# moabarar/nemar

Measured on AMD Instinct MI355X. Metric: train images/sec (256x256 A/B pairs), higher is better.
Workload: dtype f32

## Files before the change

nemar_amd/csrc/conv.hip:

```cpp
#define NEMAR_CONV_HIP
#include "common.h"
#include "conv_exact.h"
#include "conv_call.h"
#include "conv_route.h"
#include "pack_plan.h"

#ifdef NEMAR_AB
extern int g_split16_ring3;
extern int g_split16_ksplit_cap;
extern int g_narrow_fwd4;
extern int g_wg_xreg;
extern int g_register_vec4;
extern int g_overlap_per_lane;
extern int g_histogram_per_lane;
void nemar_norm_planes_debug(int bits);
#endif

int nemar_narrow_fwd(const float* x, const float* w, const float* bias, float* y, int N, int C, int H, int W, int K, int R,
                     int pad, int border, int act, float slope, float* part, size_t part_floats, hipStream_t st);
int nemar_narrow_wgrad(const float* x, const float* gy, float* gw, int N, int C, int H, int W, int K, int R, int pad,
                       int border, float* part, hipStream_t st);
void nemar_wgrad2_launch(const float* x0, int C0, const float* x1, int C1, const float* gy, float* gw, float* gb, int N,
                         int H, int W, int K, int OH, int OW, int R, int S, int stride, int pad, int pad_mode,
                         int target_blocks, bool vec_ok, int dbg, float* part, hipStream_t st);
// ... 792 lines not shown
                                       (const float*)ring_buf, gx0 ? gx0 : gx1, H, W, pad, ring_len, band, planes);
            }
        }
    if (fold && !folded) {
        const float* const add = (gx0 && !gx1) ? call.addend : nullptr;
        fold_padded(padded, gx0 ? gx0 : gx1, H, W, pad, total, add, st);
        if (add) call.addend_done = true;
    }
    }
    }
    NEMAR_CHECK_LAUNCH(what);
    return NEMAR_OK;
}

NEMAR_API size_t nemar_conv2d_bwd_weight_workspace(int N, int C, int H, int W, int K, int OH, int OW, int R, int S, int stride, int pad) {
    if (N <= 0 || C <= 0 || K <= 0 || OH <= 0 || OW <= 0 || R <= 0 || S <= 0) return 0;
    return sizeof(float) * plan_wgrad({N, C, 0, H, W, K, R, S, stride, pad, BORDER_ZERO, OH, OW}, ConvFacts::canonical()).total;
}

static int conv2d_bwd_weight(ConvCall& call, const float* x0, int C0, const float* x1, int C1, const float* gy, float* gw,
                             float* gb, int N, int H, int W, int K, int OH, int OW, int R, int S, int stride,
                             int pad, int pad_mode, void* workspace, size_t ws_bytes, void* stream) {
    NEMAR_CLEAR_HIP_ERROR();
    NEMAR_REQUIRE(x0 && gy && gw, "conv2d_bwd_weight: null pointer");
    NEMAR_REQUIRE(C0 > 0 && C1 >= 0 && (C1 == 0 || x1), "conv2d_bwd_weight: bad channel split");
    NEMAR_REQUIRE(N > 0 && H > 0 && W > 0 && K > 0 && OH > 0 && OW > 0 && R > 0 && S > 0, "conv2d_bwd_weight: bad shape");
    NEMAR_REQUIRE(pad_mode == BORDER_ZERO || (pad < H && pad < W), "conv2d_bwd_weight: reflect pad too large");
    NEMAR_REQUIRE((long long)N * OH * OW < (1ll << 31) && (long long)(C0 + C1) * H * W < (1ll << 31),
                  "conv2d_bwd_weight: problem too large for 32-bit tile indexing");
    ConvFacts f = facts_of(call, nullptr, ACT_NONE, 0.f);
    f.part = g_deterministic != 0;
    f.gy_aligned = (reinterpret_cast<uintptr_t>(gy) & 15) == 0;
    f.part_aligned = (reinterpret_cast<uintptr_t>(workspace) & 15) == 0;
    const WgradPlan P = plan_wgrad({N, C0, C1, H, W, K, R, S, stride, pad, pad_mode, OH, OW}, f);
    float* part = nullptr;
    if (g_deterministic) {
        const size_t need = sizeof(float) * P.total;
        if (!workspace || ws_bytes < need) {
            nemar_set_error("conv2d_bwd_weight: workspace %zu < %zu", workspace ? ws_bytes : (size_t)0, need);
            return NEMAR_EWORKSPACE;
        }
        part = (float*)workspace;
    }
    hipStream_t st = (hipStream_t)stream;
    const int J = (C0 + C1) * R * S;
    const char* what = "conv2d_bwd_weight";
    g_last_route = P.route;
    switch (P.sub) {
    case WgradPlan::K7:
        if (!nemar_k7_wgrad(x0, gy, gw, gb, N, C0, H, W, K, pad_mode, part, st))
            bias_grad_slabs(gy, gb, part + P.bias_off, N, K, OH * OW, st);
        what = "conv2d_bwd_weight (7x7, 16-bit pipe)";
        break;
    case WgradPlan::NARROW:
        nemar_narrow_wgrad(x0, gy, gw, N, C0, H, W, K, R, pad, pad_mode, part, st);
        if (gb) bias_grad_slabs(gy, gb, part ? part + P.bias_off : nullptr, N, K, OH * OW, st);
        what = "conv2d_bwd_weight (narrow)";
        break;
    case WgradPlan::S16G:
        nemar_s16g_wgrad(x0, C0, x1, C1, gy, gw, gb, N, H, W, K, OH, OW, R, stride, pad_mode, part, g_dbg, st);
        what = "conv2d_bwd_weight (16-bit pipe, in-kernel split)";
        break;
    case WgradPlan::SPLIT16:
        call.bias_rode = gb && call.bias_partials;
        nemar_split16_wgrad(x0, gy, gw, N, C0, H, W, K, R, pad_mode == BORDER_REFLECT ? 1 : 0, call.scratch, part, g_xcd_map,
                            R == 3 ? call.src2_planes : nullptr, (R == 3 && pad_mode == BORDER_REFLECT) ? call.x_planes : nullptr,
                            call.src_max, call.src2_max, call.bias_rode ? call.bias_partials : nullptr, gb, st);
        if (gb && !call.bias_rode) bias_grad_slabs(gy, gb, part + P.bias_off, N, K, OH * OW, st);
        what = "conv2d_bwd_weight (split-16)";
        break;
    case WgradPlan::WGRAD2:
        nemar_wgrad2_launch(x0, C0, x1, C1, gy, gw, gb, N, H, W, K, OH, OW, R, S, stride, pad, pad_mode, g_wgrad_blocks,
                            g_wgrad != 2, g_dbg, part, st);
        what = "conv2d_bwd_weight (wide)";
        break;
    case WgradPlan::WGRAD2_PADDED_GY: {
        float* gyp = part + P.gyp_off;
        const long long total = (long long)N * K * P.ohv * OW;
        hipLaunchKernelGGL(pad_planes_kernel, dim3(nemar_stream_grid(total, 256)), dim3(256), 0, st, gy, gyp, OH * OW, P.ohv * OW, total);
        nemar_wgrad2_launch(x0, C0, x1, C1, gyp, gw, gb, N, H, W, K, P.ohv, OW, R, S, stride, pad, pad_mode, g_wgrad_blocks,
                            g_wgrad != 2, g_dbg, part, st);
        what = "conv2d_bwd_weight (wide, padded gy)";
        break;
    }
    case WgradPlan::LEGACY: {
        WgradParams p;
        p.src0 = x0; p.src1 = x1; p.C0 = C0; p.C1 = C1; p.Hs = H; p.Ws = W;
        p.gy = gy; p.K = K; p.OH = OH; p.OW = OW;
        p.gw = gw; p.gb = gb; p.J = J;
        p.N = N; p.P = N * OH * OW; p.sy = stride; p.sx = stride; p.R = R; p.S = S; p.pad = pad; p.border = pad_mode;
        p.fd_ohw = make_fastdiv(OH * OW); p.fd_ow = make_fastdiv(OW);
        p.dbg = g_dbg;
        p.pix_per_split = P.pix_per_split;
        p.part = part;
        p.partb = part ? part + P.bias_off : nullptr;
        const bool wide = K > 32;
        dim3 grid(nemar_cdiv(K, wide ? 128 : 32), nemar_cdiv(J, wide ? 128 : 256), P.splits), block(256);
        if (wide) hipLaunchKernelGGL((wgrad_kernel<2, 2, 2, 2>), grid, block, 0, st, p);
        else hipLaunchKernelGGL((wgrad_kernel<1, 4, 1, 2>), grid, block, 0, st, p);
        if (part) nemar_sum_partials_pair(part, (long long)K * J, P.splits, gw, (long long)K * J, gb ? p.partb : nullptr, K, P.splits, gb, K, true, st);
    }
    }
// ... 24 lines not shown
    if (key == 26) { g_s16g_wgrad_first = value != 0; return NEMAR_OK; }
    if (key == 27) { nemar_s16g_tune(0, value); return NEMAR_OK; }
    if (key == 29) { g_s16g_wgrad = value != 0; return NEMAR_OK; }
    if (key == 31) { nemar_norm_planes_debug(value); return NEMAR_OK; }
    if (key == 32) { g_split16_ring3 = value != 0; return NEMAR_OK; }
    if (key == 33) { g_k7 = value != 0; return NEMAR_OK; }
    if (key == 36) { g_split_act = value != 0; return NEMAR_OK; }
    if (key == 43) { g_fold_small = value != 0; return NEMAR_OK; }
    if (key == 37) { g_lds_claim = value; return NEMAR_OK; }
    if (key == 38) { g_wg_xreg = value != 0; return NEMAR_OK; }
    if (key == 39) { g_split16_ksplit_cap = value < 1 ? 1 : (value > 8 ? 8 : value); return NEMAR_OK; }
    if (key == 45) { g_overlap_per_lane = value != 0; return NEMAR_OK; }
    if (key == 46) { g_histogram_per_lane = value != 0; return NEMAR_OK; }
    if (key == 44) { g_register_vec4 = value != 0; return NEMAR_OK; }
    if (key == 47) { g_pointwise_rows = value != 0; return NEMAR_OK; }
    if (key == 35) { g_dual_gy = value != 0; return NEMAR_OK; }
    if (key == 34) { nemar_split16_wgrad_tune(value); return NEMAR_OK; }
    if (key == 30) { g_s16g_fold = value != 0; return NEMAR_OK; }
    if (key == 28) { nemar_s16g_tune(1, value); return NEMAR_OK; }
    if (key == 40) { nemar_s16g_tune(2, value); return NEMAR_OK; }
    if (key == 42) { nemar_s16g_tune(4, value); return NEMAR_OK; }
    if (key == 41) { nemar_s16g_tune(3, value); return NEMAR_OK; }
    if (key == 23) { g_split16_min_mmac = value < 0 ? 0 : value; return NEMAR_OK; }
    if (key == 21) { g_split16_variant = value == 3 ? 3 : 4; return NEMAR_OK; }
    if (key == 16) { g_adir = value != 0; return NEMAR_OK; }
    if (key == 17) { g_mt8 = value; return NEMAR_OK; }
    if (key == 19) { g_narrow_fwd4 = value != 0; return NEMAR_OK; }
    if (key == 18) { g_ring = (value == 4 || value == 5) ? value : 3; return NEMAR_OK; }
    if (key == 12) { g_ksplit = value != 0; return NEMAR_OK; }
    if (key == 11) { g_nl4_scalar = value != 0; return NEMAR_OK; }
    if (key == 10) { g_deep64 = value != 0; return NEMAR_OK; }
    if (key == 7) { g_ws2_mt = (value == 1 || value == 2 || value == 4) ? value : 0; return NEMAR_OK; }
    if (key == 5) { g_wgrad_blocks = value > 0 ? value : 512; return NEMAR_OK; }
    nemar_set_error("nemar_tune: unknown key %d", key);
    return NEMAR_EINVAL;
}
#endif

static DgradPlan usual_dgrad(int N, int C, int H, int W, int K, int R, int S, int stride, int pad, int pad_mode) {
    DgradPlan P{};
    if (N <= 0 || C <= 0 || H <= 0 || W <= 0 || K <= 0 || R <= 0 || S <= 0 || stride < 1) return P;
    return plan_dgrad({N, C, 0, H, W, K, R, S, stride, pad, pad_mode}, ConvFacts::canonical());
}
static bool fusable(const DgradPlan& P) { return P.gy_planes_need != 0 && P.split16_ksplit == 1; }

NEMAR_API size_t nemar_conv2d_scratch(int N, int H, int W, int K, int C, int R, int S, int stride, int pad) {
    if (N <= 0 || H <= 0 || W <= 0 || K <= 0 || C <= 0) return 0;
    return plan_arena_bytes({N, C, 0, H, W, K, R, S, stride, pad, BORDER_ZERO});
}

NEMAR_API size_t nemar_conv2d_gy_planes_bytes(int N, int C, int H, int W, int K, int R, int S, int stride, int pad, int pad_mode) {
    return usual_dgrad(N, C, H, W, K, R, S, stride, pad, pad_mode).gy_planes_need;
}

NEMAR_API int nemar_conv2d_bwd_data_fusable(int N, int C, int H, int W, int K, int R, int S, int stride, int pad, int pad_mode) {
    return fusable(usual_dgrad(N, C, H, W, K, R, S, stride, pad, pad_mode)) ? 1 : 0;
}

NEMAR_API int nemar_conv2d_bwd_data_addend_ok(int N, int C, int H, int W, int K, int R, int S, int stride, int pad, int pad_mode) {
    const DgradPlan P = usual_dgrad(N, C, H, W, K, R, S, stride, pad, pad_mode);
    if (fusable(P)) return 1;
    if (pad_mode != BORDER_REFLECT || pad <= 0 || stride != 1 || pad >= H || pad >= W || R != S || R == 7) return 0;
    return (P.fold16 || P.fold) && plan_arena_bytes({N, C, 0, H, W, K, R, S, stride, pad, BORDER_ZERO}) == 0 ? 1 : 0;
}

NEMAR_API int nemar_last_gy_planes(void) { return g_last_gy_planes; }
// ... 127 lines not shown
```

nemar_amd/csrc/conv_route.h:

```cpp
#pragma once
#ifndef NEMAR_CONV_HIP
#error "conv_route.h holds conv.hip's own switches: include it from conv.hip only"
#endif
#include "common.h"
#include "conv_exact.h"
#include "conv_split16.h"
#include "conv_s16g.h"
#include "conv_k7.h"

bool nemar_narrow_eligible(int K, int C1, int R, int S, int stride, int N, int OH, int OW);
int nemar_narrow_wgrad_splits(int N, int C, int OH, int OW);
bool nemar_wgrad2_eligible(int K, int OH, int OW, bool gy_aligned16);
void nemar_wgrad2_plan(int K, int J, int P, int target_blocks, int* splits_out, int* pix_per_split_out);

using namespace nemar_exact;

namespace {

static NEMAR_SWITCH(int, g_split16, 1);
static NEMAR_SWITCH(long long, g_split16_min_mmac, 2000);
static NEMAR_SWITCH(int, g_split16_variant, 4);
static NEMAR_SWITCH(int, g_k7, 1);
static NEMAR_SWITCH(int, g_s16g, 1);
static NEMAR_SWITCH(long long, g_s16g_min_mmac, 30);
static NEMAR_SWITCH(int, g_s16g_wgrad, 1);
static NEMAR_SWITCH(int, g_s16g_wgrad_first, 0);
static NEMAR_SWITCH(int, g_s16g_fold, 1);
static NEMAR_SWITCH(int, g_split_act, 1);
static NEMAR_SWITCH(int, g_fold_small, 1);
static NEMAR_SWITCH(int, g_dual_gy, 1);
static NEMAR_SWITCH(int, g_reflect_aux, 1);
static NEMAR_SWITCH(int, g_deterministic, 1);
static NEMAR_SWITCH(int, g_ksplit, 1);
static NEMAR_SWITCH(int, g_narrow, 1);
static NEMAR_SWITCH(int, g_wgrad, 0);
static NEMAR_SWITCH(int, g_wgrad_blocks, 512);

enum { ROUTE_EXACT = 0, ROUTE_NARROW = 1, ROUTE_SPLIT16 = 2, ROUTE_S16G = 3, ROUTE_K7 = 4 };

struct ConvShape {
    int N, C0, C1, H, W, K, R, S, stride, pad, pad_mode;
    int oh = 0, ow = 0;
    int C() const { return C0 + C1; }
    int OH() const { return oh ? oh : (H + 2 * pad - R) / stride + 1; }
    int OW() const { return ow ? ow : (W + 2 * pad - S) / stride + 1; }
    bool refl() const { return pad_mode == BORDER_REFLECT && pad > 0; }
    long long macs() const { return (long long)N * OH() * OW() * K * C() * R * S; }
};
struct ConvFacts {
    bool bias = false;
    int act = ACT_NONE;
    float slope = 0.f;
    bool gx0 = true, gx1 = false;
    bool part = true;
    size_t scratch_bytes = 0;
    size_t gy_planes_bytes = 0;
    bool gy_aligned = true, part_aligned = true;
    static ConvFacts canonical() { ConvFacts f; f.scratch_bytes = f.gy_planes_bytes = ~(size_t)0; return f; }
};

inline void grow(size_t& a, size_t b) { if (b > a) a = b; }
constexpr int WBK = 32;
constexpr int BIAS_CHUNK = 4096;

int small_problem_split(int M, int P, int Kred) {
    const TileChoice t = igemm_tile(M, P, nemar_cdiv(Kred, BK));
    if (t.bm == 128) return 1;
    const long long tiles = (long long)nemar_cdiv(M, t.bm) * nemar_cdiv(P, t.bn);
    const int stages = nemar_cdiv(Kred, BK);
    if (tiles >= 128 || stages < 16) return 1;
    int ks = nemar_cdiv(256, (int)tiles);
    if (ks > stages / 4) ks = stages / 4;
    return ks < 1 ? 1 : ks;
}

void fwd_taps(TapTable& t, int R, int S, int pad) {
    t.n = R * S;
    for (int r = 0; r < R; ++r)
        for (int s = 0; s < S; ++s) {
            t.dy[r * S + s] = (short)(r - pad);
            t.dx[r * S + s] = (short)(s - pad);
            t.dyx[r * S + s] = ((r - pad) << 16) | ((s - pad) & 0xffff);
            t.wofs[r * S + s] = r * S + s;
        }
}

void dgrad_taps(TapTable& t, int R, int S, int pad, int stride, int ph, int pw) {
    t.n = 0;
    for (int r = 0; r < R; ++r) {
        if ((ph + pad - r) % stride != 0) continue;
// ... 260 lines not shown
        L.route = ROUTE_EXACT; L.sub = DgradPlan::EXACT;
        L.narrow = g_narrow && stride == 1 && !L.fold && !f.bias && f.act == ACT_NONE && L.mskip == 0 && !f.gx1 && R - 1 - pad >= 0 &&
                   nemar_narrow_eligible(C, 0, R, S, 1, N, H, W);
        L.split = !L.narrow && L.ksplit > 1 && !f.bias && f.act == ACT_NONE && L.mskip == 0 &&
                  (L.fold ? (f.gx0 && !f.gx1) : (!f.gx1 || (f.gx0 && !L.ring)));
        L.aux_rows = !L.narrow && L.ring && g_reflect_aux && pad == 1 && R == 3 && S == 3 && H >= 4 && W >= 8;
    }
    return L;
}

void legacy_wgrad_plan(int K, int J, int P, int* splits_out, int* pix_per_split_out) {
    const bool wide = K > 32;
    const int BM = wide ? 128 : 32, BN = wide ? 128 : 256;
    const int mt = nemar_cdiv(K, BM), jt = nemar_cdiv(J, BN);
    int splits = nemar_cdiv(1024, mt * jt);
    const int max_splits = nemar_cdiv(P, WBK * 8);
    if (splits > max_splits) splits = max_splits;
    if (splits < 1) splits = 1;
    if (splits > 65535) splits = 65535;
    *pix_per_split_out = nemar_cdiv(nemar_cdiv(P, splits), WBK) * WBK;
    *splits_out = nemar_cdiv(P, *pix_per_split_out);
}
int padded_rows(int OH, int OW) {
    int ohv = OH;
    while ((ohv * OW) % 4) ++ohv;
    return ohv;
}
bool wgrad_pad_route(int K, int OH, int OW, int pad_mode) {
    return K > 4 && (OH * OW) % 4 != 0 && pad_mode == BORDER_ZERO && g_wgrad != 1;
}

struct WgradPlan {
    int route;
    enum Sub { K7, NARROW, S16G, SPLIT16, WGRAD2, WGRAD2_PADDED_GY, LEGACY } sub;
    size_t total, bias_off, gyp_off;
    int splits, pix_per_split, ohv;
};
WgradPlan plan_wgrad(const ConvShape& s, const ConvFacts& f) {
    WgradPlan P;
    const int N = s.N, C = s.C(), H = s.H, W = s.W, K = s.K, R = s.R, S = s.S, stride = s.stride, pad = s.pad, OH = s.OH(), OW = s.OW();
    const int J = C * R * S, Pix = N * OH * OW, ohv = padded_rows(OH, OW);
    const size_t slab = (size_t)K * J, bias_parts = (size_t)N * nemar_cdiv(OH * OW, BIAS_CHUNK) * K;
    int w2_splits, legacy_splits, pad_splits = 0, pps;
    nemar_wgrad2_plan(K, J, Pix, g_wgrad_blocks, &w2_splits, &pps);
    legacy_wgrad_plan(K, J, Pix, &legacy_splits, &P.pix_per_split);
    P.total = (size_t)(w2_splits > legacy_splits ? w2_splits : legacy_splits) * (slab + K);
    if ((OH * OW) % 4 != 0 && K > 4) {
        nemar_wgrad2_plan(K, J, N * ohv * OW, g_wgrad_blocks, &pad_splits, &pps);
        grow(P.total, (size_t)pad_splits * (slab + K) + 4 + (size_t)N * K * ohv * OW);
    }
    if (K <= 4) grow(P.total, (size_t)nemar_narrow_wgrad_splits(N, C, OH, OW) * slab + bias_parts);
    if (nemar_s16g_wgrad_eligible(N, C, 0, H, W, K, OH, OW, R, S, stride, pad, BORDER_ZERO))
        grow(P.total, (size_t)nemar_s16g_wgrad_slabs_max(N, C, K, OH, W, stride) * (slab + K));
    const bool k7 = nemar_k7_wgrad_eligible(N, C, H, W, K, R, S, stride, pad);
    if (k7) grow(P.total, nemar_k7_wgrad_floats(N, C, H, W, K) + bias_parts);
    const bool wide = wide_candidates(s).wgrad;
    if (wide) grow(P.total, (size_t)nemar_split16_wgrad_splits(N, C, H, W, K, R) * slab + bias_parts);
    const bool s16g_wg = g_s16g_wgrad && f.part && s16g_worth_it(s.macs()) &&
                         nemar_s16g_wgrad_eligible(N, s.C0, s.C1, H, W, K, OH, OW, R, S, stride, pad, s.pad_mode);
    const bool split16_wg = g_split16 && g_split16_variant == 4 && f.part && s.C1 == 0 && split16_worth_it(N, OH, OW, K, C, R, S) && wide &&
                            (R == 3 || s.pad_mode == BORDER_ZERO) && f.scratch_bytes &&
                            f.scratch_bytes >= nemar_split16_wgrad_scratch_bytes(N, C, H, W, K, R);
    P.bias_off = P.gyp_off = 0; P.splits = 0; P.ohv = ohv;
    if (g_k7 && f.part && s.C1 == 0 && k7) {
        P.route = ROUTE_K7; P.sub = WgradPlan::K7; P.bias_off = nemar_k7_wgrad_floats(N, C, H, W, K);
    } else if (nemar_narrow_eligible(K, s.C1, R, S, stride, N, OH, OW) && g_narrow) {
        P.route = ROUTE_NARROW; P.sub = WgradPlan::NARROW; P.bias_off = (size_t)nemar_narrow_wgrad_splits(N, s.C0, OH, OW) * slab;
    } else if (s16g_wg && (g_s16g_wgrad_first || !split16_wg)) {
        P.route = ROUTE_S16G; P.sub = WgradPlan::S16G;
    } else if (split16_wg) {
        P.route = ROUTE_SPLIT16; P.sub = WgradPlan::SPLIT16; P.bias_off = (size_t)nemar_split16_wgrad_splits(N, C, H, W, K, R) * slab;
    } else {
        P.route = ROUTE_EXACT;
        P.gyp_off = ((size_t)pad_splits * (slab + K) + 3) & ~(size_t)3;
        const bool padded_gy = f.part && wgrad_pad_route(K, OH, OW, s.pad_mode) && nemar_wgrad2_eligible(K, ohv, OW, f.part_aligned);
        if (g_wgrad != 1 && nemar_wgrad2_eligible(K, OH, OW, f.gy_aligned)) P.sub = WgradPlan::WGRAD2;
        else if (padded_gy) P.sub = WgradPlan::WGRAD2_PADDED_GY;
        else { P.sub = WgradPlan::LEGACY; P.splits = legacy_splits; P.bias_off = (size_t)legacy_splits * slab; }
    }
    return P;
}

size_t plan_arena_bytes(const ConvShape& s) {
    const int N = s.N, C = s.C(), H = s.H, W = s.W, K = s.K, R = s.R;
    if (!g_split16 || !split16_worth_it(N, H + 2 * s.pad - R + 1, W + 2 * s.pad - s.S + 1, K, C, R, s.S)) return 0;
    const WideCandidates c = wide_candidates(s);
    size_t b = c.fwd ? nemar_split16_scratch_total(N, H, W, K, C, H, W) : 0;
    if (c.dgrad) grow(b, nemar_split16_scratch_total(N, H, W, C, K, H, W));
    if (c.wgrad) grow(b, nemar_split16_wgrad_scratch_bytes(N, C, H, W, K, R));
    return b;
}

}
```

nemar_amd/csrc/conv_split16.h:

```cpp
#pragma once
#include <hip/hip_runtime.h>
#include <stddef.h>
#include "conv_call.h"

enum { SPLIT16_ZERO = 0, SPLIT16_REFLECT = 1, SPLIT16_DGRAD_REFLECT = 2 };

bool nemar_split16_eligible(int N, int H, int W, int M, int Cred, int R, int S, int stride, int pad, int mode, int variant);
size_t nemar_split16_scratch_bytes(int N, int Cred, int H, int W);
int nemar_split16_ksplit(int N, int H, int W, int M, int Cred);
size_t nemar_split16_scratch_total(int N, int H, int W, int M, int Cred, int OH, int OW);
size_t nemar_split16_pack_bytes(int M, int Cred, int KS);
void nemar_split16_pack(const float* w, void* packed, int K, int C, int KS, int dgrad, int variant, hipStream_t st);
struct Split16Done {
    bool dual_written;
    bool epilogue_fused;
};
Split16Done nemar_split16_conv(const float* src, const void* packed, const float* bias, float* dst, int N, int H, int W, int M, int Cred,
                               int KS, int src_pad, int Hs, int Ws_src, int OH, int OW, int mode, void* scratch, int xcd_map, int variant,
                               long long* tl, void* dual_g_out, MaxWords src_max, const void* ready_planes, int ready_kind,
                               const float* addend, void* out_max, hipStream_t st);

bool nemar_split16_wgrad_eligible(int N, int C, int H, int W, int K, int R, int S, int stride, int pad);
size_t nemar_split16_wgrad_scratch_bytes(int N, int C, int H, int W, int K, int KS);
int nemar_split16_wgrad_splits(int N, int C, int H, int W, int K, int KS);
#ifdef NEMAR_AB
void nemar_split16_wgrad_tune(int one_copy);
#endif
void nemar_sum_partials_pair(const float* part_a, long long stride_a, int splits_a, float* dst_a, long long n_a,
                             const float* part_b, long long stride_b, int splits_b, float* dst_b, long long n_b, bool accumulate, hipStream_t st);
void nemar_split16_wgrad(const float* x, const float* gy, float* gw, int N, int C, int H, int W, int K, int KS, int reflect,
                         void* scratch, float* part, int xcd_map, const void* g_planes, const void* x_planes, MaxWords x_max,
                         MaxWords gy_max, const float* bias_partials, float* gb, hipStream_t st);
size_t nemar_split16_wgrad_g_bytes(int N, int H, int W, int K, int KS);
void nemar_split16_dual_split(const float* gy, void* dplanes, void* gplanes, int N, int K, int H, int W, int mode, const unsigned* maxbits,
                              int mstride, hipStream_t st);
void nemar_sum_partials(const float* part, long long stride, int splits, float* dst, long long n, bool accumulate, hipStream_t st);
void nemar_sum_partials_two(const float* part, long long stride, int splits, float* d0, float* d1, int N, int C0, int C1, int HW, hipStream_t st);
void nemar_sum_partials_act(const float* part, long long stride, int splits, float* dst, long long n, int act, float slope, hipStream_t st);

void nemar_split16_absmax(const float* x, int samples, long long per, void* out, hipStream_t st);
const unsigned* nemar_split16_source_max(const float* src, int N, long long per, MaxWords hint, unsigned* own, int* stride, hipStream_t st);

void nemar_split16_timer(int on);
int nemar_split16_timer_read(double* total_ms, double* total_flop);
```

nemar_amd/csrc/conv_split16_wgrad.hip:

```cpp
#include "common.h"
#include "conv_split16.h"

namespace {

typedef float f32x16 __attribute__((ext_vector_type(16)));
typedef _Float16 f16x8 __attribute__((ext_vector_type(8)));
typedef unsigned u32x4 __attribute__((ext_vector_type(4)));

__device__ __forceinline__ float pow2_scale(unsigned maxbits) {
    const int e = (int)((maxbits >> 23) & 255u);
    if (e == 0 || e == 255) return 1.f;
    const int se = 127 + 11 - (e - 127);
    if (se < 1 || se > 254) return 1.f;
    return __builtin_bit_cast(float, (unsigned)se << 23);
}
__device__ __forceinline__ unsigned short f16_rn(float v) {
    const _Float16 h = (_Float16)v;
    return __builtin_bit_cast(unsigned short, h);
}
__device__ __forceinline__ void split2_f16(float v, unsigned short& h, unsigned short& l) {
    h = f16_rn(v);
    const float r = v - (float)__builtin_bit_cast(_Float16, h);
    l = f16_rn(r);
}
__device__ __forceinline__ u32x4 pack8(const unsigned short* b) {
    u32x4 o;
    o[0] = (unsigned)b[0] | ((unsigned)b[1] << 16);
    o[1] = (unsigned)b[2] | ((unsigned)b[3] << 16);
    o[2] = (unsigned)b[4] | ((unsigned)b[5] << 16);
    o[3] = (unsigned)b[6] | ((unsigned)b[7] << 16);
    return o;
}
__device__ __forceinline__ int mirror(int i, int n) { return i < 0 ? -i : (i >= n ? 2 * n - 2 - i : i); }

__device__ __forceinline__ void glds16(const u32x4* g, u32x4* lds) {
    __builtin_amdgcn_global_load_lds((const __attribute__((address_space(1))) void*)g,
                                     (__attribute__((address_space(3))) void*)lds, 16, 0, 0);
}
// ... 38 lines not shown
__global__ __launch_bounds__(256) void split_wgrad_x_kernel(const float* __restrict__ x, u32x4* __restrict__ out, int N, int C, int H,
                                                            int W, int Hp, int CPR, int reflect, long long total,
                                                            const unsigned* maxbits, int mstride) {
    __shared__ float tile[64][TW + 1];
    const int CBLK = C >> 6, FX = Hp * CPR;
    const int yp = blockIdx.x % Hp, cblk = (blockIdx.x / Hp) % CBLK, n = blockIdx.x / (Hp * CBLK);
    const float scale = pow2_scale(maxbits[n * mstride]);
    int y = yp - 1;
    bool rowok = yp < H + 2;
    if (reflect) y = mirror(min(y, H), H);
    else rowok = rowok && (unsigned)y < (unsigned)H;
    const float* src = x + (((size_t)n * C + cblk * 64) * H + (rowok ? y : 0)) * W;
    for (int i = threadIdx.x; i < 64 * W; i += 256) {
        const int cc = i / W, xs = i - cc * W;
        tile[cc][xs] = rowok ? src[(size_t)cc * H * W + xs] * scale : 0.f;
    }
    __syncthreads();
    const int cc = threadIdx.x & 63;
    for (int q = threadIdx.x >> 6; q < CPR; q += 4) {
        unsigned short h[8], l[8];
        float v[8];
#pragma unroll
        for (int e = 0; e < 8; ++e) {
            const int xs = q * 8 + e - 1;
            v[e] = tile[cc][min(max(reflect ? mirror(xs, W) : xs, 0), W - 1)];
        }
#pragma unroll
        for (int e = 0; e < 8; ++e) {
            const int xp = q * 8 + e;
            const bool ok = xp < W + 2 && (reflect || (unsigned)(xp - 1) < (unsigned)W);
            split2_f16(ok ? v[e] : 0.f, h[e], l[e]);
        }
        const size_t t = (((size_t)n * CBLK + cblk) * FX + (size_t)yp * CPR + q) * 64 + cc;
        out[t] = pack8(h);
        out[total + t] = pack8(l);
    }
}

template <int TW>
__global__ __launch_bounds__(256) void split_dual_kernel(const float* __restrict__ gy, u32x4* __restrict__ dpl, u32x4* __restrict__ gpl,
                                                         int N, int K, int H, int W, int Hg, int CPR, int reflect, long long dtotal,
                                                         long long gtotal, const unsigned* maxbits, int mstride) {
    __shared__ float tile[64][TW + 1];
    const int Hp = H + 4, Ws = W + 4, KBLK = K >> 6, CG = K >> 3, F = Hg * CPR;
    const int prow = blockIdx.x % Hp, kblk = (blockIdx.x / Hp) % KBLK, n = blockIdx.x / (Hp * KBLK);
    const float scale = pow2_scale(maxbits[n * mstride]);
    const bool img = prow >= 1 && prow <= H;
    int ya = 0, yb = -1;
    bool any = img;
    if (img) ya = prow - 1;
    else if (reflect && prow == H + 2) { ya = 0; yb = 2; any = true; }
    else if (reflect && prow == H + 3) { ya = H - 3; yb = H - 1; any = true; }
    const float* src = gy + ((size_t)n * K + kblk * 64) * H * W;
    for (int i = threadIdx.x; i < 64 * W; i += 256) {
        const int kk = i / W, x = i - kk * W;
        const float a = src[((size_t)kk * H + ya) * W + x];
        const float b = src[((size_t)kk * H + max(yb, 0)) * W + x];
        tile[kk][x] = any ? (yb >= 0 ? a + b : a) * scale : 0.f;
    }
    __syncthreads();
    for (int i = threadIdx.x; i < 8 * Ws; i += 256) {
        const int cgl = i / Ws, slot = i - cgl * Ws;
        int xa = -1, xb = -1;
        if (slot >= 1 && slot <= W) xa = slot - 1;
        else if (reflect && slot == W + 2) { xa = 0; xb = 2; }
        else if (reflect && slot == W + 3) { xa = W - 3; xb = W - 1; }
// ... 13 lines not shown
    const int grow = img ? prow - 1 : (prow == 0 ? H : prow);
    if (grow < Hg && (img || prow <= H + 2)) {
        const int kk = threadIdx.x & 63;
        for (int q = threadIdx.x >> 6; q < CPR; q += 4) {
            unsigned short h[8], l[8];
            float v[8];
#pragma unroll
            for (int e = 0; e < 8; ++e) v[e] = tile[kk][min(q * 8 + e, W - 1)];
#pragma unroll
            for (int e = 0; e < 8; ++e) split2_f16((img && q * 8 + e < W) ? v[e] : 0.f, h[e], l[e]);
            const size_t t = (((size_t)n * KBLK + kblk) * F + (size_t)grow * CPR + q) * 64 + kk;
            gpl[t] = pack8(h);
            gpl[gtotal + t] = pack8(l);
        }
    }
}

struct WgParams {
    const u32x4* G;
    const u32x4* X;
    float* part;
    int N, H, W, C, K;
    int CPR, F, FX, RB, spi;
    int KBLK, CBLK;
    long long gplane16, xplane16;
    const unsigned* gmax;
    const unsigned* xmax;
    int gstride, xstride;
    int xcd;
};

template <int KS, bool ONEG, bool XREG = false>
__global__ __launch_bounds__(256) void wgrad_split16_kernel(WgParams p) {
    static_assert(!XREG || (KS == 3 && ONEG), "XREG: instantiated and measured for the 3x3 one-copy form only");

    constexpr int GC = ONEG ? 1 : KS;
    constexpr int RING = 4, NCOL = 4 * GC + 4 * KS, NCP = NCOL / 4;
    constexpr int STAGE16 = NCOL * 64;
    constexpr int NMF = 3 * KS * KS, NSL = 2 * GC + 2 * KS + NCP;
    constexpr int NPV = KS / 2;
#ifdef NEMAR_HOST_EMULATION
    __shared__ __attribute__((aligned(16))) u32x4 smem[RING * STAGE16];
#else
    extern __shared__ __attribute__((aligned(16))) u32x4 smem[];
#endif
    const int tid = threadIdx.x, wid = __builtin_amdgcn_readfirstlane(tid >> 6), lane = tid & 63;
    const int tiles = p.KBLK * p.CBLK;
    int t = blockIdx.x;
    if (p.xcd) t = (t & 7) * ((int)gridDim.x >> 3) + (t >> 3);
    const int split = t / tiles, tile = t - split * tiles;
    const int kblk = tile / p.CBLK, cblk = tile - kblk * p.CBLK;
    const int n = split / p.spi, y0 = (split - n * p.spi) * p.RB;
    const int nsteps = p.RB * p.CPR / 2, f0 = y0 * p.CPR;

    const u32x4* csrc[NCP];
#pragma unroll
    for (int q = 0; q < NCP; ++q) {
        const int i = NCP * wid + q;
        if (i < 4 * GC) {
            const int s = i >> 2, pl = (i >> 1) & 1, ch = i & 1;
            csrc[q] = p.G + (size_t)(s * 2 + pl) * p.gplane16 + (((size_t)n * p.KBLK + kblk) * p.F + f0 + ch) * 64 + lane;
        } else {
            const int j = i - 4 * GC, r = j >> 2, pl = (j >> 1) & 1, ch = j & 1;
            csrc[q] = p.X + (size_t)pl * p.xplane16 + (((size_t)n * p.CBLK + cblk) * p.FX + f0 + r * p.CPR + ch) * 64 + lane;
        }
    }
#define WG_COPIES(stage_)                                                                                               \
// ... 244 lines not shown
    NEMAR_AB_ONLY(                                                                                                                 \
    else if (KS == 3)                                                                                                              \
        hipLaunchKernelGGL((split_wgrad_g_kernel<TW_, 3>), dim3(N * KBLK * Hg), dim3(256), 0, st, gy, (u32x4*)scratch, N, K, OHg, OWg, Hg, CPR, gtotal, \
                           gmax, gstride);                                                                                         \
    else                                                                                                                           \
        hipLaunchKernelGGL((split_wgrad_g_kernel<TW_, 4>), dim3(N * KBLK * Hg), dim3(256), 0, st, gy, (u32x4*)scratch, N, K, OHg, OWg, Hg, CPR, gtotal, \
                           gmax, gstride);)                                                                                        \
    if (!have_x)                                                                                                                   \
        hipLaunchKernelGGL((split_wgrad_x_kernel<TW_>), dim3(N * CBLK * Hx), dim3(256), 0, st, x, X, N, C, H, W, Hx, CPR, reflect, xtotal, \
                           xmax, xstride);
    if (W <= 64) { WG_SPLIT(64) } else if (W <= 128) { WG_SPLIT(128) } else { WG_SPLIT(256) }
#undef WG_SPLIT
    WgParams p;
    p.G = G; p.X = X; p.part = part;
    p.N = N; p.H = H; p.W = W; p.C = C; p.K = K;
    p.CPR = CPR; p.F = Hg * CPR; p.FX = Hx * CPR;
    p.RB = rows_per_split(N, Hg, CPR, KBLK * CBLK);
    p.spi = Hg / p.RB;
    p.KBLK = KBLK; p.CBLK = CBLK;
    p.gplane16 = gtotal; p.xplane16 = xtotal;
    p.gmax = gmax; p.xmax = xmax; p.gstride = gstride; p.xstride = xstride;
    const int splits = N * p.spi, grid = splits * KBLK * CBLK;
    p.xcd = (xcd_map && grid % 8 == 0 && (grid / 8) % (KBLK * CBLK) == 0) ? 1 : 0;
    NEMAR_AB_ONLY(if (KS == 3 && oneg && !g_wg_xreg) wg_launch<3, true, false>(grid, p, st); else)
    if (KS == 3 && oneg) wg_launch<3, true, true>(grid, p, st);
    else if (oneg) wg_launch<4, true>(grid, p, st);
#ifdef NEMAR_AB
    else if (KS == 3) wg_launch<3, false>(grid, p, st);
    else wg_launch<4, false>(grid, p, st);
#endif
    nemar_sum_partials_pair(part, (long long)K * C * KS * KS, splits, gw, (long long)K * C * KS * KS, bias_partials, K, N,
                            bias_partials ? gb : nullptr, K, true, st);
}
```

nemar_amd/csrc/reduce.hip:

```cpp
#include "common.h"

namespace {

typedef float f32x4 __attribute__((ext_vector_type(4)));

template <bool VEC>
__device__ __forceinline__ void sum_general_body(f32x4 (*red)[17], const float* __restrict__ part, long long stride, int splits,
                                                 float* __restrict__ dst, long long n, int accumulate, int act, float slope,
                                                 unsigned bx, unsigned gx) {
    const int tx = threadIdx.x & 15, ty = threadIdx.x >> 4;
    const long long cols = VEC ? (n >> 2) : n;
    for (long long c0 = (long long)bx * 16; c0 < cols; c0 += (long long)gx * 16) {
        const long long c = c0 + tx;
        f32x4 acc = {0.f, 0.f, 0.f, 0.f};
        if (c < cols) {
            for (int s = ty; s < splits; s += 16) {
                const float* q = part + (long long)s * stride;
                if (VEC) acc += *reinterpret_cast<const f32x4*>(q + 4 * c);
                else acc[0] += q[c];
            }
        }
        red[ty][tx] = acc;
        __syncthreads();
        if (ty == 0 && c < cols) {
            f32x4 t = red[0][tx];
#pragma unroll
            for (int y = 1; y < 16; ++y) t += red[y][tx];
            if (VEC) {
                f32x4* d = reinterpret_cast<f32x4*>(dst + 4 * c);
                if (accumulate) t += *d;
                if (act) {
#pragma unroll
                    for (int e = 0; e < 4; ++e) t[e] = t[e] > 0.f ? t[e] : (act == 1 ? 0.f : t[e] * slope);
                }
                *d = t;
            } else {
                if (accumulate) t[0] += dst[c];
                if (act) t[0] = t[0] > 0.f ? t[0] : (act == 1 ? 0.f : t[0] * slope);
                dst[c] = t[0];
            }
        }
        __syncthreads();
    }
}
template <bool VEC>
__global__ __launch_bounds__(256) void sum_partials_kernel(const float* __restrict__ part, long long stride, int splits,
                                                           float* __restrict__ dst, long long n, int accumulate, int act,
                                                           float slope) {
    __shared__ f32x4 red[16][17];
    sum_general_body<VEC>(red, part, stride, splits, dst, n, accumulate, act, slope, blockIdx.x, gridDim.x);
}

__device__ __forceinline__ void sum_few_body(const float* __restrict__ part, long long stride, int splits, float* __restrict__ dst, long long n,
                                             int accumulate, int act, float slope, unsigned bx, unsigned gx) {
    const long long cols = n >> 2;
    for (long long c = (long long)bx * 256 + threadIdx.x; c < cols; c += (long long)gx * 256) {
        f32x4 v[16];
#pragma unroll
        for (int s = 0; s < 16; ++s)
            v[s] = *reinterpret_cast<const f32x4*>(part + (long long)(s < splits ? s : 0) * stride + 4 * c);
        f32x4 t = {0.f, 0.f, 0.f, 0.f};
        t += v[0];
#pragma unroll
        for (int s = 1; s < 16; ++s)
            if (s < splits) t += v[s];
        f32x4* d = reinterpret_cast<f32x4*>(dst + 4 * c);
        if (accumulate) t += *d;
        if (act) {
#pragma unroll
            for (int e = 0; e < 4; ++e) t[e] = t[e] > 0.f ? t[e] : (act == 1 ? 0.f : t[e] * slope);
        }
        *d = t;
    }
}
__global__ __launch_bounds__(256) void sum_partials_few_kernel(const float* __restrict__ part, long long stride, int splits,
                                                               float* __restrict__ dst, long long n, int accumulate, int act, float slope) {
    sum_few_body(part, stride, splits, dst, n, accumulate, act, slope, blockIdx.x, gridDim.x);
}

struct SumJob {
    const float* part; long long stride; int splits; float* dst; long long n; int accumulate; int kind; unsigned blocks;
};
__global__ __launch_bounds__(256) void sum_partials_pair_kernel(SumJob a, SumJob b) {
    __shared__ f32x4 red[16][17];
    const bool first = blockIdx.x < a.blocks;
    const SumJob& j = first ? a : b;
    const unsigned bx = first ? blockIdx.x : blockIdx.x - a.blocks;
    if (j.kind == 0) sum_few_body(j.part, j.stride, j.splits, j.dst, j.n, j.accumulate, 0, 0.f, bx, j.blocks);
    else if (j.kind == 1) sum_general_body<true>(red, j.part, j.stride, j.splits, j.dst, j.n, j.accumulate, 0, 0.f, bx, j.blocks);
    else sum_general_body<false>(red, j.part, j.stride, j.splits, j.dst, j.n, j.accumulate, 0, 0.f, bx, j.blocks);
}

__global__ __launch_bounds__(256) void sum_partials_two_kernel(const float* __restrict__ part, long long stride, int splits, float* __restrict__ d0,
                                                               float* __restrict__ d1, int C0, int C1, int HW, long long total) {
    const int C = C0 + C1;
    for (long long idx = (long long)blockIdx.x * 256 + threadIdx.x; idx < total; idx += (long long)gridDim.x * 256) {
        const long long n = idx / ((long long)C * HW);
        const int r = (int)(idx - n * C * HW), c = r / HW, px = r - c * HW;
        float t = 0.f;
        for (int sidx = 0; sidx < splits; ++sidx) t += part[(long long)sidx * stride + idx];
        if (c < C0) d0[((size_t)n * C0 + c) * HW + px] = t;
        else d1[((size_t)n * C1 + (c - C0)) * HW + px] = t;
    }
}

__global__ __launch_bounds__(256) void sum_partials_fold_kernel(const float* __restrict__ part, long long stride, int splits, float* __restrict__ gx,
                                                                int H, int W, int pad, long long total, const float* __restrict__ addend) {
    __shared__ float val[16][9][17];
    const int Hp = H + 2 * pad, Wp = W + 2 * pad;
    const int tx = threadIdx.x & 15, ty = threadIdx.x >> 4;
    for (long long idx0 = (long long)blockIdx.x * 16; idx0 < total; idx0 += (long long)gridDim.x * 16) {
        const long long idx = idx0 + tx;
        const bool live = idx < total;
        const long long cidx = live ? idx : total - 1;
        const int w = (int)(cidx % W);
        const long long t = cidx / W;
        const int h = (int)(t % H);
        const long long nc = t / H;
        const int y0 = h + pad, x0 = w + pad;
        const int y1 = (h >= 1 && h <= pad) ? pad - h : -1, y2 = (h <= H - 2 && h >= H - 1 - pad) ? 2 * (H - 1) - h + pad : -1;
        const int x1 = (w >= 1 && w <= pad) ? pad - w : -1, x2 = (w <= W - 2 && w >= W - 1 - pad) ? 2 * (W - 1) - w + pad : -1;
        const int ya = y1 >= 0 ? y1 : y0, yb = y2 >= 0 ? y2 : y0, xa = x1 >= 0 ? x1 : x0, xb = x2 >= 0 ? x2 : x0;
// ... 70 lines not shown
}

static void sum_partials_launch(const float* part, long long stride, int splits, float* dst, long long n, bool accumulate, int act, float slope,
                                hipStream_t st) {
    const bool vec = (n & 3) == 0 && (stride & 3) == 0 && ((reinterpret_cast<uintptr_t>(part) | reinterpret_cast<uintptr_t>(dst)) & 15) == 0;
    const long long cols = vec ? (n >> 2) : n;
    long long blocks = (cols + 15) / 16;
    if (blocks > 256 * 16) blocks = 256 * 16;
    if (blocks < 1) blocks = 1;
    if (vec && splits >= 1 && splits <= 16) {
        long long fb = (cols + 255) / 256;
        if (fb > 2048) fb = 2048;
        hipLaunchKernelGGL(sum_partials_few_kernel, dim3((unsigned)fb), dim3(256), 0, st, part, stride, splits, dst, n, accumulate ? 1 : 0, act,
                           slope);
    } else if (vec)
        hipLaunchKernelGGL((sum_partials_kernel<true>), dim3((unsigned)blocks), dim3(256), 0, st, part, stride, splits, dst, n,
                           accumulate ? 1 : 0, act, slope);
    else
        hipLaunchKernelGGL((sum_partials_kernel<false>), dim3((unsigned)blocks), dim3(256), 0, st, part, stride, splits, dst, n,
                           accumulate ? 1 : 0, act, slope);
}

void nemar_sum_partials(const float* part, long long stride, int splits, float* dst, long long n, bool accumulate, hipStream_t st) {
    sum_partials_launch(part, stride, splits, dst, n, accumulate, 0, 0.f, st);
}

void nemar_sum_partials_pair(const float* part_a, long long stride_a, int splits_a, float* dst_a, long long n_a,
                             const float* part_b, long long stride_b, int splits_b, float* dst_b, long long n_b, bool accumulate, hipStream_t st) {
    if (!part_b || !dst_b) { nemar_sum_partials(part_a, stride_a, splits_a, dst_a, n_a, accumulate, st); return; }
    const SumJob a = sum_job(part_a, stride_a, splits_a, dst_a, n_a, accumulate), b = sum_job(part_b, stride_b, splits_b, dst_b, n_b, accumulate);
    hipLaunchKernelGGL(sum_partials_pair_kernel, dim3(a.blocks + b.blocks), dim3(256), 0, st, a, b);
}

void nemar_sum_partials_act(const float* part, long long stride, int splits, float* dst, long long n, int act, float slope, hipStream_t st) {
    sum_partials_launch(part, stride, splits, dst, n, false, act, slope, st);
}
```

Before: 287.9.

## Route 4x4 stride-2 weight gradients through split-16 as space-to-depth 2x2

Adds a weight-gradient path for 4x4 stride-2 pad-1 convolutions. The input is rearranged space-to-depth into 4C channels, so the existing split-16 half-precision matrix-core kernel can run it as a 2x2 stride-1 problem. A permuted partial-sum reduction then maps the result back to the original weight layout. It is meant to replace the slower exact/wide path for these downsampling layers, at the cost of an extra packing kernel, more workspace and new layout-remapping code.

```diff
diff --git a/nemar_amd/csrc/conv.hip b/nemar_amd/csrc/conv.hip
--- a/nemar_amd/csrc/conv.hip
+++ b/nemar_amd/csrc/conv.hip
@@ -848,6 +848,7 @@
     f.part = g_deterministic != 0;
     f.gy_aligned = (reinterpret_cast<uintptr_t>(gy) & 15) == 0;
     f.part_aligned = (reinterpret_cast<uintptr_t>(workspace) & 15) == 0;
+    f.gw_aligned = (reinterpret_cast<uintptr_t>(gw) & 15) == 0;
     const WgradPlan P = plan_wgrad({N, C0, C1, H, W, K, R, S, stride, pad, pad_mode, OH, OW}, f);
     float* part = nullptr;
     if (g_deterministic) {
@@ -884,6 +885,13 @@
                             call.src_max, call.src2_max, call.bias_rode ? call.bias_partials : nullptr, gb, st);
         if (gb && !call.bias_rode) bias_grad_slabs(gy, gb, part + P.bias_off, N, K, OH * OW, st);
         what = "conv2d_bwd_weight (split-16)";
+        break;
+    case WgradPlan::SPLIT16_S2D:
+        call.bias_rode = gb && call.bias_partials;
+        nemar_split16_wgrad_s2d(x0, gy, gw, N, C0, H, W, K, part + P.gyp_off, part, g_xcd_map, call.src_max, call.src2_max,
+                                call.bias_rode ? call.bias_partials : nullptr, gb, st);
+        if (gb && !call.bias_rode) bias_grad_slabs(gy, gb, part + P.bias_off, N, K, OH * OW, st);
+        what = "conv2d_bwd_weight (split-16, 4x4 stride 2 as 2x2)";
         break;
     case WgradPlan::WGRAD2:
         nemar_wgrad2_launch(x0, C0, x1, C1, gy, gw, gb, N, H, W, K, OH, OW, R, S, stride, pad, pad_mode, g_wgrad_blocks,
@@ -974,6 +982,8 @@
     if (key == 10) { g_deep64 = value != 0; return NEMAR_OK; }
     if (key == 7) { g_ws2_mt = (value == 1 || value == 2 || value == 4) ? value : 0; return NEMAR_OK; }
     if (key == 5) { g_wgrad_blocks = value > 0 ? value : 512; return NEMAR_OK; }
+    if (key == 49) { g_wgrad_s2d_min_mmac = value < 0 ? 0 : value; return NEMAR_OK; }
+    if (key == 48) { g_wgrad_s2d = value != 0; return NEMAR_OK; }
     nemar_set_error("nemar_tune: unknown key %d", key);
     return NEMAR_EINVAL;
 }
diff --git a/nemar_amd/csrc/conv_route.h b/nemar_amd/csrc/conv_route.h
--- a/nemar_amd/csrc/conv_route.h
+++ b/nemar_amd/csrc/conv_route.h
@@ -35,6 +35,8 @@
 static NEMAR_SWITCH(int, g_narrow, 1);
 static NEMAR_SWITCH(int, g_wgrad, 0);
 static NEMAR_SWITCH(int, g_wgrad_blocks, 512);
+static NEMAR_SWITCH(long long, g_wgrad_s2d_min_mmac, 6000);
+static NEMAR_SWITCH(int, g_wgrad_s2d, 1);
 
 enum { ROUTE_EXACT = 0, ROUTE_NARROW = 1, ROUTE_SPLIT16 = 2, ROUTE_S16G = 3, ROUTE_K7 = 4 };
 
@@ -56,6 +58,7 @@
     size_t scratch_bytes = 0;
     size_t gy_planes_bytes = 0;
     bool gy_aligned = true, part_aligned = true;
+    bool gw_aligned = true;
     static ConvFacts canonical() { ConvFacts f; f.scratch_bytes = f.gy_planes_bytes = ~(size_t)0; return f; }
 };
 
@@ -382,7 +385,7 @@
 
 struct WgradPlan {
     int route;
-    enum Sub { K7, NARROW, S16G, SPLIT16, WGRAD2, WGRAD2_PADDED_GY, LEGACY } sub;
+    enum Sub { K7, NARROW, S16G, SPLIT16, SPLIT16_S2D, WGRAD2, WGRAD2_PADDED_GY, LEGACY } sub;
     size_t total, bias_off, gyp_off;
     int splits, pix_per_split, ohv;
 };
@@ -406,6 +409,12 @@
     if (k7) grow(P.total, nemar_k7_wgrad_floats(N, C, H, W, K) + bias_parts);
     const bool wide = wide_candidates(s).wgrad;
     if (wide) grow(P.total, (size_t)nemar_split16_wgrad_splits(N, C, H, W, K, R) * slab + bias_parts);
+    const bool s2d = R == 4 && S == 4 && stride == 2 && pad == 1 && OH == H / 2 && OW == W / 2 && nemar_split16_wgrad_s2d_eligible(N, C, H, W, K) &&
+                     s.macs() >= g_wgrad_s2d_min_mmac * 1000000ll;
+    const size_t s2d_planes_off = s2d ? ((size_t)nemar_split16_wgrad_s2d_splits(N, C, H, W, K) * slab + bias_parts + 3) & ~(size_t)3 : 0;
+    if (s2d) grow(P.total, s2d_planes_off + (nemar_split16_wgrad_s2d_plane_bytes(N, C, H, W, K) + 3) / 4);
+    const bool s2d_wg = g_wgrad_s2d != 0 && g_split16 != 0 && g_split16_variant == 4 && f.part && s.C1 == 0 && s2d && s.pad_mode == BORDER_ZERO &&
+                        s16g_worth_it(s.macs()) && f.part_aligned && f.gw_aligned;
     const bool s16g_wg = g_s16g_wgrad && f.part && s16g_worth_it(s.macs()) &&
                          nemar_s16g_wgrad_eligible(N, s.C0, s.C1, H, W, K, OH, OW, R, S, stride, pad, s.pad_mode);
     const bool split16_wg = g_split16 && g_split16_variant == 4 && f.part && s.C1 == 0 && split16_worth_it(N, OH, OW, K, C, R, S) && wide &&
@@ -420,6 +429,9 @@
         P.route = ROUTE_S16G; P.sub = WgradPlan::S16G;
     } else if (split16_wg) {
         P.route = ROUTE_SPLIT16; P.sub = WgradPlan::SPLIT16; P.bias_off = (size_t)nemar_split16_wgrad_splits(N, C, H, W, K, R) * slab;
+    } else if (s2d_wg) {
+        P.route = ROUTE_SPLIT16; P.sub = WgradPlan::SPLIT16_S2D;
+        P.bias_off = (size_t)nemar_split16_wgrad_s2d_splits(N, C, H, W, K) * slab; P.gyp_off = s2d_planes_off;
     } else {
         P.route = ROUTE_EXACT;
         P.gyp_off = ((size_t)pad_splits * (slab + K) + 3) & ~(size_t)3;
diff --git a/nemar_amd/csrc/conv_split16.h b/nemar_amd/csrc/conv_split16.h
--- a/nemar_amd/csrc/conv_split16.h
+++ b/nemar_amd/csrc/conv_split16.h
@@ -32,6 +32,13 @@
                          void* scratch, float* part, int xcd_map, const void* g_planes, const void* x_planes, MaxWords x_max,
                          MaxWords gy_max, const float* bias_partials, float* gb, hipStream_t st);
 size_t nemar_split16_wgrad_g_bytes(int N, int H, int W, int K, int KS);
+bool nemar_split16_wgrad_s2d_eligible(int N, int C, int H, int W, int K);
+size_t nemar_split16_wgrad_s2d_plane_bytes(int N, int C, int H, int W, int K);
+int nemar_split16_wgrad_s2d_splits(int N, int C, int H, int W, int K);
+void nemar_split16_wgrad_s2d(const float* x, const float* gy, float* gw, int N, int C, int H, int W, int K, void* planes, float* part,
+                             int xcd_map, MaxWords x_max, MaxWords gy_max, const float* bias_partials, float* gb, hipStream_t st);
+void nemar_sum_partials_pair_s2d(const float* part_a, long long stride_a, int splits_a, float* dst_a, long long n_a,
+                                 const float* part_b, long long stride_b, int splits_b, float* dst_b, long long n_b, bool accumulate, hipStream_t st);
 void nemar_split16_dual_split(const float* gy, void* dplanes, void* gplanes, int N, int K, int H, int W, int mode, const unsigned* maxbits,
                               int mstride, hipStream_t st);
 void nemar_sum_partials(const float* part, long long stride, int splits, float* dst, long long n, bool accumulate, hipStream_t st);
diff --git a/nemar_amd/csrc/conv_split16_wgrad.hip b/nemar_amd/csrc/conv_split16_wgrad.hip
--- a/nemar_amd/csrc/conv_split16_wgrad.hip
+++ b/nemar_amd/csrc/conv_split16_wgrad.hip
@@ -4,6 +4,7 @@
 namespace {
 
 typedef float f32x16 __attribute__((ext_vector_type(16)));
+typedef float f32x4 __attribute__((ext_vector_type(4)));
 typedef _Float16 f16x8 __attribute__((ext_vector_type(8)));
 typedef unsigned u32x4 __attribute__((ext_vector_type(4)));
 
@@ -108,6 +109,47 @@
             split2_f16(ok ? v[e] : 0.f, h[e], l[e]);
         }
         const size_t t = (((size_t)n * CBLK + cblk) * FX + (size_t)yp * CPR + q) * 64 + cc;
+        out[t] = pack8(h);
+        out[total + t] = pack8(l);
+    }
+}
+
+template <int TW, bool VEC>
+__global__ __launch_bounds__(256) void split_wgrad_x_s2d_kernel(const float* __restrict__ x, u32x4* __restrict__ out, int N, int C, int H,
+                                                                int W, int Hx, int CPR, long long total, const unsigned* maxbits,
+                                                                int mstride) {
+    __shared__ float tile[32][TW + 2];
+    const int CBLK = C >> 4, FX = Hx * CPR;
+    const int i = blockIdx.x % Hx, cblk = (blockIdx.x / Hx) % CBLK, n = blockIdx.x / (Hx * CBLK);
+    const float scale = pow2_scale(maxbits[n * mstride]);
+    const float* src = x + ((size_t)n * C + cblk * 16) * H * W;
+    if (VEC) {
+        const int W4 = W >> 2;
+        for (int t = threadIdx.x; t < 32 * W4; t += 256) {
+            const int r = t / W4, x4 = t - r * W4, y = 2 * i + (r & 1) - 1;
+            const bool ok = (unsigned)y < (unsigned)H;
+            const f32x4 v = *reinterpret_cast<const f32x4*>(src + ((size_t)(r >> 1) * H + min(max(y, 0), H - 1)) * W + 4 * x4);
+#pragma unroll
+            for (int e = 0; e < 4; ++e) tile[r][4 * x4 + e] = ok ? v[e] * scale : 0.f;
+        }
+    } else {
+        for (int t = threadIdx.x; t < 32 * W; t += 256) {
+            const int r = t / W, xs = t - r * W, y = 2 * i + (r & 1) - 1;
+            const bool ok = (unsigned)y < (unsigned)H;
+            const float v = src[((size_t)(r >> 1) * H + min(max(y, 0), H - 1)) * W + xs];
+            tile[r][xs] = ok ? v * scale : 0.f;
+        }
+    }
+    __syncthreads();
+    const int cc = threadIdx.x & 63, r = cc >> 1, q = cc & 1;
+    for (int ch = threadIdx.x >> 6; ch < CPR; ch += 4) {
+        unsigned short h[8], l[8];
+        float v[8];
+#pragma unroll
+        for (int e = 0; e < 8; ++e) v[e] = tile[r][min(max(2 * (ch * 8 + e) + q - 1, 0), W - 1)];
+#pragma unroll
+        for (int e = 0; e < 8; ++e) split2_f16((unsigned)(2 * (ch * 8 + e) + q - 1) < (unsigned)W ? v[e] : 0.f, h[e], l[e]);
+        const size_t t = (((size_t)n * CBLK + cblk) * FX + (size_t)i * CPR + ch) * 64 + cc;
         out[t] = pack8(h);
         out[total + t] = pack8(l);
     }
@@ -187,7 +229,7 @@
 
 template <int KS, bool ONEG, bool XREG = false>
 __global__ __launch_bounds__(256) void wgrad_split16_kernel(WgParams p) {
-    static_assert(!XREG || (KS == 3 && ONEG), "XREG: instantiated and measured for the 3x3 one-copy form only");
+    static_assert(!XREG || ((KS == 3 || KS == 2) && ONEG), "XREG: instantiated and measured for the 3x3 and 2x2 one-copy forms only");
 
     constexpr int GC = ONEG ? 1 : KS;
     constexpr int RING = 4, NCOL = 4 * GC + 4 * KS, NCP = NCOL / 4;
@@ -498,3 +540,66 @@
     nemar_sum_partials_pair(part, (long long)K * C * KS * KS, splits, gw, (long long)K * C * KS * KS, bias_partials, K, N,
                             bias_partials ? gb : nullptr, K, true, st);
 }
+
+static int s2d_cpr(int W) { return (W / 2 + 1 + 7) / 8; }
+static int s2d_rows(int H) { return (H / 2 + 3) / 4 * 4; }
+
+bool nemar_split16_wgrad_s2d_eligible(int N, int C, int H, int W, int K) {
+    if (H % 2 || W % 2 || H < 4 || W < 4 || W > SPLIT_MAXW || N > 256) return false;
+    if (K % 64 || C % 16 || 4 * C < 128 || K < 128) return false;
+    const int CPR = s2d_cpr(W), Hg = s2d_rows(H);
+    if (rows_per_split(N, Hg, CPR, (K / 64) * (C / 16)) == 0) return false;
+    if ((long long)N * (4 * C > K ? 4 * C : K) * (Hg + 1) * CPR * 64 >= (1ll << 31)) return false;
+    return true;
+}
+
+size_t nemar_split16_wgrad_s2d_plane_bytes(int N, int C, int H, int W, int K) {
+    const int CPR = s2d_cpr(W), Hg = s2d_rows(H);
+    return ((size_t)2 * N * K * Hg * CPR + (size_t)2 * N * 4 * C * (Hg + 1) * CPR) * 16 + 2048;
+}
+
+int nemar_split16_wgrad_s2d_splits(int N, int C, int H, int W, int K) {
+    const int CPR = s2d_cpr(W), Hg = s2d_rows(H);
+    const int rb = rows_per_split(N, Hg, CPR, (K / 64) * (C / 16));
+    return rb ? N * (Hg / rb) : 0;
+}
+
+void nemar_split16_wgrad_s2d(const float* x, const float* gy, float* gw, int N, int C, int H, int W, int K, void* planes, float* part,
+                             int xcd_map, MaxWords x_max, MaxWords gy_max, const float* bias_partials, float* gb, hipStream_t st) {
+    const int OH = H / 2, OW = W / 2, CPR = s2d_cpr(W), Hg = s2d_rows(H), Hx = Hg + 1, KBLK = K / 64, CBLK = C / 16;
+    const long long gtotal = (long long)N * K * Hg * CPR, xtotal = (long long)N * 4 * C * Hx * CPR;
+    u32x4* const G = (u32x4*)planes;
+    u32x4* const X = G + 2 * gtotal;
+    unsigned* const mw = (unsigned*)(X + 2 * xtotal);
+    int gstride = 0, xstride = 0;
+    const unsigned* const gmax = nemar_split16_source_max(gy, N, (long long)K * OH * OW, gy_max, mw, &gstride, st);
+    const unsigned* const xmax = nemar_split16_source_max(x, N, (long long)C * H * W, x_max, mw + 256, &xstride, st);
+#define WG_S2D_G(TW_)                                                                                                              \
+    hipLaunchKernelGGL((split_wgrad_g_kernel<TW_, 1>), dim3(N * KBLK * Hg), dim3(256), 0, st, gy, G, N, K, OH, OW, Hg, CPR, gtotal, gmax, gstride);
+    if (OW <= 64) { WG_S2D_G(64) } else { WG_S2D_G(128) }
+#undef WG_S2D_G
+    const bool vec = W % 4 == 0 && (reinterpret_cast<uintptr_t>(x) & 15) == 0;
+#define WG_S2D_X(TW_)                                                                                                              \
+    if (vec)                                                                                                                       \
+        hipLaunchKernelGGL((split_wgrad_x_s2d_kernel<TW_, true>), dim3(N * CBLK * Hx), dim3(256), 0, st, x, X, N, C, H, W, Hx, CPR, xtotal, xmax, \
+                           xstride);                                                                                               \
+    else                                                                                                                           \
+        hipLaunchKernelGGL((split_wgrad_x_s2d_kernel<TW_, false>), dim3(N * CBLK * Hx), dim3(256), 0, st, x, X, N, C, H, W, Hx, CPR, xtotal, xmax, \
+                           xstride);
+    if (W <= 64) { WG_S2D_X(64) } else if (W <= 128) { WG_S2D_X(128) } else { WG_S2D_X(256) }
+#undef WG_S2D_X
+    WgParams p;
+    p.G = G; p.X = X; p.part = part;
+    p.N = N; p.H = H; p.W = W; p.C = 4 * C; p.K = K;
+    p.CPR = CPR; p.F = Hg * CPR; p.FX = Hx * CPR;
+    p.RB = rows_per_split(N, Hg, CPR, KBLK * CBLK);
+    p.spi = Hg / p.RB;
+    p.KBLK = KBLK; p.CBLK = CBLK;
+    p.gplane16 = gtotal; p.xplane16 = xtotal;
+    p.gmax = gmax; p.xmax = xmax; p.gstride = gstride; p.xstride = xstride;
+    const int splits = N * p.spi, grid = splits * KBLK * CBLK;
+    p.xcd = (xcd_map && grid % 8 == 0 && (grid / 8) % (KBLK * CBLK) == 0) ? 1 : 0;
+    wg_launch<2, true, true>(grid, p, st);
+    nemar_sum_partials_pair_s2d(part, (long long)K * C * 16, splits, gw, (long long)K * C * 16, bias_partials, K, N,
+                                bias_partials ? gb : nullptr, K, true, st);
+}
diff --git a/nemar_amd/csrc/reduce.hip b/nemar_amd/csrc/reduce.hip
--- a/nemar_amd/csrc/reduce.hip
+++ b/nemar_amd/csrc/reduce.hip
@@ -4,7 +4,16 @@
 
 typedef float f32x4 __attribute__((ext_vector_type(4)));
 
-template <bool VEC>
+typedef float f32x2 __attribute__((ext_vector_type(2)));
+template <bool PERM>
+__device__ __forceinline__ f32x4 slab_column(const float* __restrict__ q, long long c) {
+    if (!PERM) return *reinterpret_cast<const f32x4*>(q + 4 * c);
+    const float* const g = q + 16 * (c >> 2) + 8 * (c & 1) + 2 * ((c >> 1) & 1);
+    const f32x2 lo = *reinterpret_cast<const f32x2*>(g), hi = *reinterpret_cast<const f32x2*>(g + 4);
+    return f32x4{lo[0], hi[0], lo[1], hi[1]};
+}
+
+template <bool VEC, bool PERM = false>
 __device__ __forceinline__ void sum_general_body(f32x4 (*red)[17], const float* __restrict__ part, long long stride, int splits,
                                                  float* __restrict__ dst, long long n, int accumulate, int act, float slope,
                                                  unsigned bx, unsigned gx) {
@@ -16,7 +25,7 @@
         if (c < cols) {
             for (int s = ty; s < splits; s += 16) {
                 const float* q = part + (long long)s * stride;
-                if (VEC) acc += *reinterpret_cast<const f32x4*>(q + 4 * c);
+                if (VEC) acc += slab_column<PERM>(q, c);
                 else acc[0] += q[c];
             }
         }
@@ -51,6 +60,7 @@
     sum_general_body<VEC>(red, part, stride, splits, dst, n, accumulate, act, slope, blockIdx.x, gridDim.x);
 }
 
+template <bool PERM = false>
 __device__ __forceinline__ void sum_few_body(const float* __restrict__ part, long long stride, int splits, float* __restrict__ dst, long long n,
                                              int accumulate, int act, float slope, unsigned bx, unsigned gx) {
     const long long cols = n >> 2;
@@ -58,7 +68,7 @@
         f32x4 v[16];
 #pragma unroll
         for (int s = 0; s < 16; ++s)
-            v[s] = *reinterpret_cast<const f32x4*>(part + (long long)(s < splits ? s : 0) * stride + 4 * c);
+            v[s] = slab_column<PERM>(part + (long long)(s < splits ? s : 0) * stride, c);
         f32x4 t = {0.f, 0.f, 0.f, 0.f};
         t += v[0];
 #pragma unroll
@@ -88,6 +98,8 @@
     const unsigned bx = first ? blockIdx.x : blockIdx.x - a.blocks;
     if (j.kind == 0) sum_few_body(j.part, j.stride, j.splits, j.dst, j.n, j.accumulate, 0, 0.f, bx, j.blocks);
     else if (j.kind == 1) sum_general_body<true>(red, j.part, j.stride, j.splits, j.dst, j.n, j.accumulate, 0, 0.f, bx, j.blocks);
+    else if (j.kind == 3) sum_few_body<true>(j.part, j.stride, j.splits, j.dst, j.n, j.accumulate, 0, 0.f, bx, j.blocks);
+    else if (j.kind == 4) sum_general_body<true, true>(red, j.part, j.stride, j.splits, j.dst, j.n, j.accumulate, 0, 0.f, bx, j.blocks);
     else sum_general_body<false>(red, j.part, j.stride, j.splits, j.dst, j.n, j.accumulate, 0, 0.f, bx, j.blocks);
 }
 
@@ -224,6 +236,16 @@
     hipLaunchKernelGGL(sum_partials_pair_kernel, dim3(a.blocks + b.blocks), dim3(256), 0, st, a, b);
 }
 
+void nemar_sum_partials_pair_s2d(const float* part_a, long long stride_a, int splits_a, float* dst_a, long long n_a,
+                                 const float* part_b, long long stride_b, int splits_b, float* dst_b, long long n_b, bool accumulate, hipStream_t st) {
+    SumJob a = sum_job(part_a, stride_a, splits_a, dst_a, n_a, accumulate);
+    a.kind += 3;
+    SumJob b = a;
+    b.blocks = 0;
+    if (part_b && dst_b) b = sum_job(part_b, stride_b, splits_b, dst_b, n_b, accumulate);
+    hipLaunchKernelGGL(sum_partials_pair_kernel, dim3(a.blocks + b.blocks), dim3(256), 0, st, a, b);
+}
+
 void nemar_sum_partials_act(const float* part, long long stride, int splits, float* dst, long long n, int act, float slope, hipStream_t st) {
     sum_partials_launch(part, stride, splits, dst, n, false, act, slope, st);
 }
```

New measurement: 289.9, median of 6. About the same (+0.7%).
